# edwindn/rl-agent-for-qubit-array-tuning

Measured on NVIDIA B200. Metric: ground_state_pixels_per_s, higher is better.
Workload: dtype f64

## Files before the change

rl-agent-for-qubit-array-tuning_b200/csrc/qd_api.cu:

```cuda
#include <cuda_runtime.h>
#include <stdarg.h>
#include <stdio.h>
#include <string.h>

#include <new>
#include <stdlib.h>

#include <algorithm>
#include <chrono>
#include <vector>

#include "qd_kernels.cuh"
#include "qd_tunnel.cuh"
#include "qd_tunnel_noda.cuh"
#include "qd_tunnel_enum.cuh"
#include "qd_normalise.cuh"

static_assert(sizeof(qd_scan) == 480, "qd_scan must be 480 bytes (multiple of 16 for the TMA bulk copy)");
static_assert(sizeof(qd_scan) % 16 == 0, "qd_scan size");

struct qd_ctx {
  int device = 0;
  int sm_count = 0;
  char err[512] = {0};
// ... 181 lines not shown
int validate_launch(qd_ctx* ctx, int n_type, unsigned flags, const void* n_out) {
  if (!ctx) return fail(nullptr, QD_ERR_INVALID, "ctx is NULL");
  if (!ctx->have_models) return fail(ctx, QD_ERR_STATE, "qd_set_models has not been called");
  if (n_type < QD_N_NONE || n_type > QD_N_F64) return fail(ctx, QD_ERR_INVALID, "bad n_type %d", n_type);
  if (n_type != QD_N_NONE && !n_out) return fail(ctx, QD_ERR_INVALID, "n_out is NULL but n_type != QD_N_NONE");
  if ((flags & QD_FLAG_THERMAL) && n_type == QD_N_U8)
    return fail(ctx, QD_ERR_INVALID, "QD_FLAG_THERMAL yields non-integer occupations: use QD_N_F32/F64 or QD_N_NONE");
  if ((flags & QD_FLAG_LATCH) && (flags & QD_FLAG_LATCH_EXACT) &&
      ((flags & QD_FLAG_THERMAL) || ctx->L.algorithm == QD_ALG_TUNNEL))
    return fail(ctx, QD_ERR_UNSUPPORTED,
                "QD_FLAG_LATCH_EXACT: exact-compare latching of non-integer occupations (thermal / tunnel path) is not supported");
  if (ctx->L.algorithm == QD_ALG_TUNNEL && n_type == QD_N_U8)
    return fail(ctx, QD_ERR_INVALID, "the tunnel path yields non-integer occupations <n>: use QD_N_F32/F64 or QD_N_NONE");
  return QD_OK;
}

struct KernelConfig { int device; const void* fn; size_t smem; };
KernelConfig g_kernel_config[512];
int g_n_kernel_config = 0;

int configure_kernel(qd_ctx* ctx, const void* fn, size_t smem) {
  int at = -1;
  for (int i = 0; i < g_n_kernel_config; ++i)
    if (g_kernel_config[i].fn == fn && g_kernel_config[i].device == ctx->device) { at = i; break; }
  if (at >= 0 && g_kernel_config[at].smem >= smem) return QD_OK;
  const size_t want = std::max<size_t>(smem, 48 * 1024);
  QD_CUDA(ctx, cudaFuncSetAttribute(fn, cudaFuncAttributeMaxDynamicSharedMemorySize, (int)want));
  if (at < 0) QD_CUDA(ctx, cudaFuncSetAttribute(fn, cudaFuncAttributePreferredSharedMemoryCarveout, 100));
  if (at < 0 && g_n_kernel_config < 512) at = g_n_kernel_config++;
  if (at >= 0) g_kernel_config[at] = KernelConfig{ctx->device, fn, want};
  return QD_OK;
}

int order_after_last_launch(qd_ctx* ctx, cudaStream_t stream) {
  if (ctx->have_last && ctx->last_stream != stream) QD_CUDA(ctx, cudaStreamWaitEvent(stream, ctx->last_launch, 0));
  return QD_OK;
}
int mark_launch(qd_ctx* ctx, cudaStream_t stream) {
  QD_CUDA(ctx, cudaEventRecord(ctx->last_launch, stream));
  ctx->last_stream = stream;
  ctx->have_last = true;
  return QD_OK;
}

int launch(qd_ctx* ctx, int n_scan, const qd_scan* d_scans, int max_ny, const double* d_points, float* d_z, void* d_n,
           int n_type, unsigned flags, cudaStream_t stream, int rows_cap = 0, const qd_scan* h_one = nullptr) {
  {
    const int rc0 = order_after_last_launch(ctx, stream);
    if (rc0) return rc0;
  }
  const bool fast = use_fast_kernel(ctx->L, flags, d_points != nullptr);
  kernel_fn fn = fast ? pick_fast(ctx->L.n_dot) : pick_kernel(ctx->L, flags, d_points != nullptr);
  if (!fn) return fail(ctx, QD_ERR_UNSUPPORTED, "no kernel for n_dot=%d algorithm=%d", ctx->L.n_dot, ctx->L.algorithm);
  qd::KArgs a;
  memset(&a, 0, sizeof(a));
  a.nbar = nullptr;
  if (ctx->L.algorithm == QD_ALG_TUNNEL) {
    const int N = ctx->L.n_dot;
    kernel_fn gs = pick_tunnel_gs(N);
    if (!gs) return fail(ctx, QD_ERR_UNSUPPORTED, "tunnel path needs 2..8 dots, got %d", N);
    int rc = grow(ctx, &ctx->d_nbar, &ctx->nbar_cap, (size_t)ctx->up_pixels * N * sizeof(double));
    if (rc) return rc;
    qd::KArgs g;
    memset(&g, 0, sizeof(g));
    g.L = ctx->L; g.records = ctx->d_records; g.scans = d_scans; g.points = d_points; g.z_out = nullptr;
    g.n_out = nullptr; g.nbar = ctx->d_nbar; g.n_scan = n_scan; g.n_type = QD_N_NONE; g.flags = flags;
    g.status = ctx->d_status;
    g.topt = 7;
    if (const char* e = getenv("QDSIM_TUNNEL_OPT")) g.topt = atoi(e) & 7;
    const long long max_pix = ctx->up_max_pix;
    const char* mono_e = getenv("QDSIM_TUNNEL_MONO");
    const bool mono = mono_e && mono_e[0] == '1';
    if (mono) {
      g.slot_bytes = qd::qd_tunnel_slot_bytes(ctx->L);
      const long long want_items = (long long)ctx->sm_count * 12 * 4;
      long long ppi = ((long long)n_scan * max_pix) / want_items;
      if (ppi < 1) ppi = 1;
      if (ppi > 64) ppi = 64;
      g.rows_per_item = (int)ppi;
      g.items_per_scan = (int)((max_pix + ppi - 1) / ppi);
      const long long items = (long long)n_scan * g.items_per_scan;
      const int gw = (items < (long long)ctx->sm_count * 4) ? 1 : 4;
      long long ggrid = (items + gw - 1) / gw;
      if (ggrid > 0x7fffffffLL) ggrid = 0x7fffffffLL;
      const size_t gsmem = (size_t)g.slot_bytes * gw;
      rc = configure_kernel(ctx, (const void*)gs, gsmem);
      if (rc) return rc;
      gs<<<(unsigned)ggrid, gw * 32, gsmem, stream>>>(g);
      QD_CUDA(ctx, cudaGetLastError());
      ctx->launches += 1;
    } else {
      kernel_fn kr = pick_tunnel_relax(N), ks = pick_tunnel_select(N), ke = pick_tunnel_eigen(N);
      long long chunk_pix = 8LL << 20;
      if (const char* e = getenv("QDSIM_TUNNEL_CHUNK_PIX")) chunk_pix = atoll(e) > 0 ? atoll(e) : chunk_pix;
      long long spc = chunk_pix / max_pix;
      if (spc < 1) spc = 1;
      if (spc > n_scan) spc = n_scan;
      rc = grow(ctx, &ctx->d_tfloor, &ctx->tfloor_cap, (size_t)spc * max_pix * 8);
      if (rc) return rc;
      rc = grow(ctx, &ctx->d_tkeys, &ctx->tkeys_cap, (size_t)spc * max_pix * 256);
      if (rc) return rc;
      rc = grow(ctx, &ctx->d_tpot, &ctx->tpot_cap, (size_t)spc * max_pix * 128);
      if (rc) return rc;
      g.tfloor = ctx->d_tfloor;
      g.tpot = ctx->d_tpot;
      g.tkeys = ctx->d_tkeys;
// ... 800 lines not shown
```

rl-agent-for-qubit-array-tuning_b200/csrc/qd_kernels.cuh:

```cuda
#pragma once
#include <math.h>

#include "qd_device.cuh"
#include "qd_layout.h"

namespace qd {

struct KArgs {
  qd_layout L;
  const double* __restrict__ records;
  const qd_scan* __restrict__ scans;
  const double* __restrict__ points;
  float* __restrict__ z_out;
  void* __restrict__ n_out;
  double* __restrict__ nbar;
  unsigned* status;
  unsigned char* tfloor;
  unsigned long long* tkeys;
  double* tpot;
  long long tstride;
  int topt;
  int fixup;
  int mark_ppi;
  float e2_kappa, e2_qsafe, e2_tol;
// ... 17 lines not shown
  int b = L.rec_doubles * 8 + (int)sizeof(qd_scan) + QD_DER_DOUBLES * 8 + 16;
  if (L.algorithm == QD_ALG_DEFAULT || L.algorithm == QD_ALG_THRESHOLDED) b += QD_PC_DOUBLES * 8;
  if (L.algorithm == QD_ALG_BRUTE_FORCE) b += QD_BF_DOUBLES * 8;
  return (b + 127) & ~127;
}

#ifndef QD_MIN_BLOCKS
#define QD_MIN_BLOCKS 3
#endif
#ifndef QD_CTA_WARPS
#define QD_CTA_WARPS 4
#endif
constexpr int QD_PC_WAYS = 8;

template <int N>
__device__ __forceinline__ void matvec_smem(const double* __restrict__ M, const double (&x)[N], double (&y)[N]) {
  if constexpr (N % 2 == 0) {
#pragma unroll
    for (int i = 0; i < N; ++i) {
      double s0 = 0.0, s1 = 0.0;
#pragma unroll
      for (int j = 0; j < N; j += 2) {
        const double2 m = *reinterpret_cast<const double2*>(M + i * N + j);
        s0 = fma(m.x, x[j], s0);
        s1 = fma(m.y, x[j + 1], s1);
      }
      y[i] = s0 + s1;
    }
  } else {
#pragma unroll
    for (int i = 0; i < N; ++i) {
      double s0 = 0.0;
#pragma unroll
      for (int j = 0; j < N; ++j) s0 = fma(M[i * N + j], x[j], s0);
      y[i] = s0;
    }
  }
}
struct ProjCache {
  double* aff;
  const double* gsrc;
  double* lin_s;
  uint32_t* keys;
  uint32_t* meta;
  double* mats;
  double* aug;
  int mat_stride;
};

template <int N>
__device__ __noinline__ int proj_cache_build(const ProjCache& pc, const double* __restrict__ cdd, unsigned S, int lane) {
  constexpr int W = 2 * N;
  double* A = pc.aug;
  for (int e = lane; e < N * W; e += 32) {
    const int r = e / W, c = e - r * W;
    double v;
    if (c < N) v = (((S >> r) & 1u) && ((S >> c) & 1u)) ? cdd[r * N + c] : (r == c ? 1.0 : 0.0);
    else v = (r == c - N) ? 1.0 : 0.0;
    A[e] = v;
  }
  __syncwarp();
  for (int k = 0; k < N; ++k) {
    if (!((S >> k) & 1u)) continue;
    const double inv = 1.0 / A[k * W + k];
    double rowk[(N * W + 31) / 32], fr[(N * W + 31) / 32];
#pragma unroll
    for (int t = 0; t < (N * W + 31) / 32; ++t) {
      const int e = lane + 32 * t;
      if (e < N * W) {
        const int r = e / W, c = e - r * W;
        rowk[t] = A[k * W + c] * inv;
        fr[t] = A[r * W + k];
      }
    }
    __syncwarp();
#pragma unroll
    for (int t = 0; t < (N * W + 31) / 32; ++t) {
      const int e = lane + 32 * t;
      if (e < N * W) {
        const int r = e / W;
        A[e] = (r == k) ? rowk[t] : A[e] - fr[t] * rowk[t];
      }
    }
    __syncwarp();
  }
  const int slot = (int)pc.meta[1];
  double* P = pc.mats + slot * pc.mat_stride;
  for (int e = lane; e < N * N; e += 32) {
    const int i = e / N, j = e - i * N;
    double v = (i == j) ? 1.0 : 0.0;
    if ((S >> j) & 1u) {
      for (int q = 0; q < N; ++q)
        if ((S >> q) & 1u) v -= cdd[i * N + q] * A[q * W + N + j];
    }
    if ((S >> i) & 1u) v = 0.0;
    P[e] = v;
  }
  __syncwarp();
  if (pc.gsrc != nullptr && lane < 24) {
    const int t = lane >> 3, i = lane & 7;
    double acc = 0.0;
    if (i < N) {
      const double* src = pc.gsrc + 8 * t;
      for (int j = 0; j < N; ++j) acc = fma(P[i * N + j], src[j], acc);
    }
    pc.aff[slot * 24 + lane] = acc;
// ... 466 lines not shown
};
__device__ __forceinline__ ItemWindow item_window(const KArgs& a, int part, int nx, int ny) {
  const int cparts = a.col_parts > 1 ? a.col_parts : 1;
  const int rpart = part / cparts, cpart = part - rpart * cparts;
  ItemWindow w;
  w.row0 = rpart * a.rows_per_item;
  w.row1 = min(ny, w.row0 + a.rows_per_item);
  const int n_chunk_x = (nx + 31) >> 5;
  w.cx0 = ((n_chunk_x * cpart) / cparts) << 5;
  w.cx1 = min(nx, ((n_chunk_x * (cpart + 1)) / cparts) << 5);
  w.empty = w.row0 >= ny || w.cx0 >= w.cx1;
  return w;
}

template <int N>
__device__ __forceinline__ void item_affine_forms(const KArgs& a, const double* rec, const qd_scan* sc, double* der, int lane,
                                                  bool check_overflow = true) {
  const qd_layout& L = a.L;
  const int NV = L.n_volt;
  if (lane <= N) {
    const double* arow = (lane < N) ? rec + L.o_a + lane * NV : rec + L.o_sa;
    double s0 = 0.0, sx = 0.0, sy = 0.0;
    for (int k = 0; k < NV; ++k) {
      const double c = arow[k];
      s0 = fma(c, sc->v0[k], s0);
      sx = fma(c, sc->dx[k], sx);
      sy = fma(c, sc->dy[k], sy);
    }
    if (lane < N) {
      der[lane] = s0; der[8 + lane] = sx; der[16 + lane] = sy;
      const double gmax = s0 + fmax(sx * (double)(sc->nx - 1), 0.0) + fmax(sy * (double)(sc->ny - 1), 0.0);
      const bool replaced = (a.flags & QD_FLAG_RADIAL) && sc->rad_mode == 2;
      if (check_overflow && !replaced && !(gmax < 252.0) && a.status)
        *reinterpret_cast<volatile unsigned*>(a.status) = QD_STATUS_OCC_OVERFLOW;
    } else { der[24] = s0; der[25] = sx; der[26] = sy; }
  }
}

struct PixelDraws {
  float z_white, z_rad, u_latch, u_tele;
};
__device__ __forceinline__ PixelDraws pixel_draws(bool need_rng, uint64_t seed, long long pix) {
  PixelDraws d = {0.f, 0.f, 0.f, 0.f};
  if (need_rng) {
    const Philox4 w = philox4x32_10(seed, (uint64_t)pix, 0u);
    box_muller(w.w0, w.w1, d.z_white, d.z_rad);
    d.u_latch = u24(w.w2);
    d.u_tele = u24(w.w3);
  }
  return d;
}

template <typename TakeHeld>
__device__ __forceinline__ void latch_chunk(uint64_t& key, uint64_t& held_key, unsigned todo, float u_latch, const double* rec,
                                            const qd_layout& L, int lane, TakeHeld&& take_held) {
  while (true) {
    const unsigned diff = __ballot_sync(0xffffffffu, key != held_key) & todo;
    if (!diff) break;
    const int i = __ffs(diff) - 1;
    const uint64_t ck = shfl_u64(key, i);
    const uint64_t x = ck ^ held_key;
    const uint64_t nz = (((x & 0x7f7f7f7f7f7f7f7fULL) + 0x7f7f7f7f7f7f7f7fULL) | x) & 0x8080808080808080ULL;
    const int ndiff = __popcll(nz);
    double p_acc = 2.0;
    if (ndiff == 1) {
      p_acc = rec[L.o_pleads + ((__ffsll((long long)nz) - 1) >> 3)];
    } else if (ndiff == 2) {
      const int d0 = (__ffsll((long long)nz) - 1) >> 3;
      const int d1 = (63 - __clzll((long long)nz)) >> 3;
      p_acc = rec[L.o_pinter + d0 * 8 + d1];
    }
    const unsigned from_i = ~((1u << i) - 1u);
    const unsigned same = __ballot_sync(0xffffffffu, key == ck) & todo & from_i;
    const unsigned brk = ~same & from_i & todo;
    const unsigned run = same & ~(brk ? (~0u << (__ffs(brk) - 1)) : 0u);
    const unsigned acc = __ballot_sync(0xffffffffu, (double)u_latch < p_acc) & run;
    const int acl = acc ? __ffs(acc) - 1 : 32;
    const unsigned rejected = run & ((acl >= 32) ? ~0u : ((1u << acl) - 1u));
    if ((rejected >> lane) & 1u) key = held_key;
    take_held(i, rejected, acl);
    if (acl < 32) held_key = ck;
    const int done_to = (acl < 32) ? acl : (31 - __clz(run));
    todo &= ~((2u << done_to) - 1u);
  }
}

__device__ __forceinline__ uint32_t tele_start(bool f_carry, uint64_t seed, int iy, const double* par) {
  if (f_carry) return 0u;
  const Philox4 wr = philox4x32_10(seed, (uint64_t)iy, 1u);
  return ((double)u24(wr.w0) < par[QD_PAR_TELE_STAT]) ? 1u : 0u;
}

__device__ __forceinline__ float sensor_lorentz10(double x0, double xs) {
  float zs = 0.f;
#pragma unroll
  for (int k = -5; k < 5; ++k) {
    const float xk = (float)fma((double)k, xs, x0);
    zs += rcp_approx(fmaf(xk, xk, 1.0f));
  }
  return zs;
}

__device__ __forceinline__ float radial_amp(const qd_scan* sc, double fx, double fy) {
  const float vx = (float)fma(fx, sc->rad_dx, sc->rad_x0);
  const float vy = (float)fma(fy, sc->rad_dy, sc->rad_y0);
  const float dist = sqrtf(fmaf(vx, vx, vy * vy));
  return fminf(fmaxf((float)sc->rad_alpha * (dist - (float)sc->rad_zero_radius), 0.0f), (float)sc->rad_max_amp);
}

template <int N, int ALG, bool THERMAL, bool POINTS>
__global__ void __launch_bounds__(QD_CTA_WARPS * 32, QD_MIN_BLOCKS) qd_scan_kernel(const KArgs a) {
  extern __shared__ __align__(128) unsigned char qd_smem[];
  const int lane = threadIdx.x & 31;
  const int warp = threadIdx.x >> 5;
  const int warps_per_cta = blockDim.x >> 5;
  const qd_layout& L = a.L;
  const int NV = L.n_volt;

  unsigned char* slot = qd_smem + (size_t)warp * a.slot_bytes;
  double* rec = reinterpret_cast<double*>(slot);
  qd_scan* sc = reinterpret_cast<qd_scan*>(slot + (size_t)L.rec_doubles * 8);
  double* der = reinterpret_cast<double*>(slot + (size_t)L.rec_doubles * 8 + sizeof(qd_scan));
  uint64_t* bar = reinterpret_cast<uint64_t*>(der + QD_DER_DOUBLES);
// ... 118 lines not shown
        if (!replace) {
          if constexpr (!POINTS) {
            const double fx = (double)ixc, fy = (double)iy;
#pragma unroll
            for (int j = 0; j < N; ++j) g[j] = fma(fy, d_gy[j], fma(fx, d_gx[j], d_g0[j]));
            us = fma(fy, d_us[2], fma(fx, d_us[1], d_us[0]));
          } else {
            const double* __restrict__ v = a.points + (size_t)pix * NV;
#pragma unroll
            for (int j = 0; j < N; ++j) g[j] = 0.0;
            us = 0.0;
            for (int k = 0; k < NV; ++k) {
              const double vk = v[k];
#pragma unroll
              for (int j = 0; j < N; ++j) g[j] = fma(rec[L.o_a + j * NV + k], vk, g[j]);
              us = fma(rec[L.o_sa + k], vk, us);
            }
            if constexpr (ALG != QD_ALG_BRUTE_FORCE) {
              bool big = false;
#pragma unroll
              for (int j = 0; j < N; ++j) big |= !(g[j] < 252.0);
              if (big && a.status) *reinterpret_cast<volatile unsigned*>(a.status) = QD_STATUS_OCC_OVERFLOW;
            }
          }

          if constexpr (ALG == QD_ALG_TUNNEL) {
            const double* __restrict__ src = a.nbar + (size_t)(pix0 + pix) * N;
#pragma unroll
            for (int j = 0; j < N; ++j) nd[j] = src[j];
          } else if constexpr (ALG == QD_ALG_BRUTE_FORCE) {
            double gp[N];
            if constexpr (!POINTS) {
              const double fx = (double)ixc, fy = (double)iy;
#pragma unroll
              for (int l = 0; l < N; ++l) { const int j = bf_pm[l]; gp[l] = fma(fy, d_gy[j], fma(fx, d_gx[j], d_g0[j])); }
            } else {
#pragma unroll
              for (int l = 0; l < N; ++l) gp[l] = g[l];
            }
            ground_state_brute<N, THERMAL>(gp, rec, L, bf_ud, bf_pm, kT, nd);
          }
          else ground_state_box<N, THERMAL, !POINTS>(g, rec, L, pc, lane, L.algorithm == QD_ALG_THRESHOLDED, kT, (double)ixc, (double)iy, nd);

          if (latch_on) {
            const bool integral = ALG != QD_ALG_TUNNEL && kT <= 0.0;
            uint64_t key = pack_key<N>(nd, integral);
            const uint64_t key_free = key;
            unsigned todo = vmask;
            if (!have_held) {
              held_key = shfl_u64(key, 0);
              todo &= ~1u;
              have_held = true;
            }
            latch_chunk(key, held_key, todo, rnd.u_latch, rec, L, lane, [&](int i, unsigned rejected, int) {
              if (rejected && !integral) {
                const int src = (i > 0) ? i - 1 : 0;
#pragma unroll
                for (int j = 0; j < N; ++j) {
                  const double prev = shfl_f64(nd[j], src);
                  const double held = (i > 0) ? prev : d_carry[j];
                  if ((rejected >> lane) & 1u) nd[j] = held;
                }
              }
            });
            if (integral) {
              if (key != key_free) {
#pragma unroll
                for (int j = 0; j < N; ++j) nd[j] = (double)(int)((unsigned)(key >> (8 * j)) & 0xffu);
              }
            } else {
              const int last = 31 - __clz(vmask);
              if (lane == last) {
#pragma unroll
                for (int j = 0; j < N; ++j) d_carry[j] = nd[j];
              }
              __syncwarp();
            }
          }

          double noise_in = 0.0, noise_out = 0.0;
          if (f_noise) {
            const double wn = par[QD_PAR_WHITE] * (double)rnd.z_white;
            if (f_white_out) noise_out = wn; else noise_in = wn;
            const double tamp = par[QD_PAR_TELE_AMP];
            if (tamp != 0.0) {
              if (!tele_init) {
                tele_state = tele_start(f_carry, seed, iy, par);
                tele_init = true;
              }
              const uint32_t flip0 = ((double)rnd.u_tele < par[QD_PAR_P01]) ? 1u : 0u;
              const uint32_t flip1 = ((double)rnd.u_tele < par[QD_PAR_P10]) ? 1u : 0u;
              uint32_t fn = valid ? ((0u ^ flip0) | ((1u ^ flip1) << 1)) : 2u;
#pragma unroll
              for (int d = 1; d < 32; d <<= 1) {
                const uint32_t other = __shfl_up_sync(0xffffffffu, fn, d);
                if (lane >= d) fn = compose2(fn, other);
              }
              const uint32_t st = (fn >> tele_state) & 1u;
              tele_state = __shfl_sync(0xffffffffu, st, 31);
              noise_in += tamp * (double)st;
            }
          }
          if (f_pink && par[QD_PAR_PINK] != 0.0) {
            if (!pink_init) {
              const Philox4 ws = philox4x32_10(seed, (uint64_t)iy, 3u);
              float s0, s1, s2, s3;
              box_muller(ws.w0, ws.w1, s0, s1);
// ... 55 lines not shown
            }
            z = zs + noise_out;
          } else {
            z = (double)sensor_lorentz10(x0, xs) + noise_out;
          }
          if (f_radial && sc->rad_mode == 1) z = fma((double)rnd.z_rad, (double)radial_amp(sc, (double)ixc, (double)iy), z);
          zf = (float)z;
        } else {
          zf = rnd.z_rad;
#pragma unroll
          for (int j = 0; j < N; ++j) nd[j] = 0.0;
        }

        if (valid) {
          const long long o = pix0 + (long long)iy * nx + ix;
          if (a.z_out) a.z_out[o] = zf;
          if (a.n_type == QD_N_U8) {
            unsigned char* p = reinterpret_cast<unsigned char*>(a.n_out) + o * N;
            if constexpr (N == 8) {
              uint64_t k = 0;
#pragma unroll
              for (int j = 0; j < N; ++j) k |= (uint64_t)(unsigned char)min(255, (int)nd[j]) << (8 * j);
              *reinterpret_cast<uint64_t*>(p) = k;
            } else if constexpr (N == 4) {
              uint32_t k = 0;
#pragma unroll
              for (int j = 0; j < N; ++j) k |= (uint32_t)(unsigned char)min(255, (int)nd[j]) << (8 * j);
              *reinterpret_cast<uint32_t*>(p) = k;
            } else if constexpr (N == 2) {
              const uint16_t k = (uint16_t)((unsigned char)min(255, (int)nd[0]) | ((unsigned char)min(255, (int)nd[1]) << 8));
              *reinterpret_cast<uint16_t*>(p) = k;
            } else {
#pragma unroll
              for (int j = 0; j < N; ++j) p[j] = (unsigned char)min(255, (int)nd[j]);
            }
          } else if (a.n_type == QD_N_F32) {
            float* p = reinterpret_cast<float*>(a.n_out) + o * N;
#pragma unroll
            for (int j = 0; j < N; ++j) p[j] = (float)nd[j];
          } else if (a.n_type == QD_N_F64) {
            double* p = reinterpret_cast<double*>(a.n_out) + o * N;
#pragma unroll
            for (int j = 0; j < N; ++j) p[j] = nd[j];
          }
        }
      }
    }
    __syncwarp();
  }
}


#ifndef QD_FAST_MIN_BLOCKS
#define QD_FAST_MIN_BLOCKS 4
#endif
constexpr int QD_FAST_DER = 32;
constexpr int QD_FAST_PC = 64 + 8 * 16 + 8 + 8 * 32 + QD_PC_WAYS * 24;

__host__ __device__ inline int qd_fast_slot_bytes(const qd_layout& L) {
  const int b = L.rec_doubles * 8 + (int)sizeof(qd_scan) + (QD_FAST_DER + 32 + QD_FAST_PC) * 8 + 16;
  return (b + 127) & ~127;
}

template <int N>
__global__ void __launch_bounds__(QD_CTA_WARPS * 32, QD_FAST_MIN_BLOCKS) qd_scan_fast_kernel(const KArgs a) {
  extern __shared__ __align__(128) unsigned char qd_smem[];
  const int lane = threadIdx.x & 31;
  const int warp = threadIdx.x >> 5;
  const int warps_per_cta = blockDim.x >> 5;
  const qd_layout& L = a.L;

  unsigned char* slot = qd_smem + (size_t)warp * a.slot_bytes;
  double* rec = reinterpret_cast<double*>(slot);
  qd_scan* sc = reinterpret_cast<qd_scan*>(slot + (size_t)L.rec_doubles * 8);
  double* der = reinterpret_cast<double*>(slot + (size_t)L.rec_doubles * 8 + sizeof(qd_scan));
  double* d_g0 = der;
  double* d_gx = der + 8;
  double* d_gy = der + 16;
  double* d_us = der + 24;
  double* d_sg = der + 27;
  double* swt = der + QD_FAST_DER;
  ProjCache pc;
  pc.mats = swt + 32;
  pc.aug = pc.mats + 64;
  pc.keys = reinterpret_cast<uint32_t*>(pc.aug + 8 * 16);
  pc.meta = pc.keys + QD_PC_WAYS;
  pc.lin_s = pc.aug + 8 * 16 + 8;
  pc.aff = pc.lin_s + 8 * 32;
  pc.gsrc = der;
  pc.mat_stride = 0;
  uint64_t* bar = reinterpret_cast<uint64_t*>(pc.aff + QD_PC_WAYS * 24);

  if (lane == 0) mbar_init(bar, 1);
  __syncwarp();
  uint32_t phase = 0;

  const bool f_latch = a.flags & QD_FLAG_LATCH;
  const bool f_noise = a.flags & QD_FLAG_NOISE;
  const bool f_radial = a.flags & QD_FLAG_RADIAL;
  const bool f_carry = a.flags & QD_FLAG_CARRY_ROWS;
  const bool f_white_out = a.flags & QD_FLAG_WHITE_ON_OUTPUT;
  const bool thresholded = L.algorithm == QD_ALG_THRESHOLDED;
  const uint32_t rec_bytes = (uint32_t)L.rec_doubles * 8u;
  const double* __restrict__ cinv = rec + L.o_cinv;
  const double* __restrict__ Q = rec + L.o_q;
  const double* __restrict__ spos = rec + L.o_spos;
  const double* __restrict__ sneg = rec + L.o_sneg;
  const double* __restrict__ sw = rec + L.o_sw;
  const double* par = rec + L.o_par;

  const long long total_items = (long long)a.n_scan * a.items_per_scan;
  for (long long item = (long long)blockIdx.x * warps_per_cta + warp; item < total_items;
       item += (long long)gridDim.x * warps_per_cta) {
    const int scan_id = (int)(item / a.items_per_scan);
    const int part = (int)(item - (long long)scan_id * a.items_per_scan);
    const qd_scan* gscan = a.scans + scan_id;

    stage_item(a, gscan, rec_bytes, rec, sc, bar, phase, lane, a.use_one);
    if (lane == 0) { pc.meta[0] = 0u; pc.meta[1] = 0u; }

    const int nx = sc->nx, ny = sc->ny;
    const ItemWindow w = item_window(a, part, nx, ny);
    if (w.empty) { __syncwarp(); continue; }
    const int row0 = w.row0, row1 = w.row1, cx0 = w.cx0, cx1 = w.cx1;

    item_affine_forms<N>(a, rec, sc, der, lane);
    {
      double t = 0.0;
      const int h = lane & 15;
#pragma unroll
      for (int q = 0; q < 4; ++q) {
        const int p = (lane < 16) ? q : q + 4;
        if (p < N && ((h >> q) & 1)) t += sw[N - 1 - p];
      }
      swt[lane] = t;
    }
    __syncwarp();
    if (lane < 3) {
      double t = 0.0;
      for (int j = 0; j < N; ++j) t = fma(sw[j], der[8 * lane + j], t);
      d_sg[lane] = t;
    }
    __syncwarp();

    const bool latch_on = f_latch && par[QD_PAR_LATCH] != 0.0;
    const bool replace = f_radial && sc->rad_mode == 2;
    const uint64_t seed = sc->seed;
    const long long pix0 = sc->pix_offset;
    const double inv_gamma = 1.0 / sc->peak_width;
    const double css = rec[L.o_css];
    const bool need_rng = f_noise || latch_on || (f_radial && sc->rad_mode != 0);

    uint64_t held_key = 0;
    double held_sn = 0.0;
    bool have_held = false;
    uint32_t tele_state = 0;
    bool tele_init = false;

    for (int iy = row0; iy < row1; ++iy) {
      if (!f_carry) { have_held = false; tele_init = false; }
      for (int c0 = cx0; c0 < cx1; c0 += 32) {
        const int ix = c0 + lane;
        const bool valid = ix < nx;
        const int ixc = valid ? ix : nx - 1;
        const long long pix = (long long)iy * nx + ixc;
        const unsigned vmask = __ballot_sync(0xffffffffu, valid);
        const double fx = (double)ixc, fy = (double)iy;
        const PixelDraws rnd = pixel_draws(need_rng, seed, pix);

        uint64_t key = 0;
        float zf;
        if (!replace) {
          double sn;
          {
            double g[N], nc[N];
            int sgn = 0;
#pragma unroll
            for (int j = 0; j < N; ++j) {
              g[j] = fma(fy, d_gy[j], fma(fx, d_gx[j], d_g0[j]));
              nc[j] = g[j];
              sgn |= __double2hiint(g[j]);
            }
            if (__any_sync(0xffffffffu, sgn < 0)) relax_lcp<N, true>(g, rec + L.o_cdd, pc, lane, fx, fy, nc);
            double r[N], lin[N];
            unsigned fixmask = 0, fixval = 0;
            uint32_t klo = 0, khi = 0;
            sn = 0.0;
#pragma unroll
            for (int j = 0; j < N; ++j) {
              const double fj = floor(nc[j]);
              r[j] = fj - g[j];
              sn = fma(sw[j], fj, sn);
              const uint32_t fi = (uint32_t)__double2int_rz(fj) & 0xffu;
              if (j < 4) klo |= fi << (8 * j); else khi |= fi << (8 * (j - 4));
              if (thresholded) {
                const double frac = nc[j] - fj;
                if (!(fabs(frac - 0.5) < 0.5 * par[QD_PAR_THRESHOLD])) {
                  fixmask |= 1u << (N - 1 - j);
                  if (floor(nc[j] + 0.5) - fj == 1.0) fixval |= 1u << (N - 1 - j);
                }
              }
            }
            key = ((uint64_t)khi << 32) | klo;
            matvec_smem<N>(cinv, r, lin);
            double* __restrict__ ls = pc.lin_s + lane;
            unsigned zmask = 0, omask = 0;
#pragma unroll
            for (int j = 0; j < N; ++j) {
              const unsigned bit = 1u << (N - 1 - j);
              const double l2 = lin[j] + lin[j];
              ls[(N - 1 - j) * 32] = l2;
              const double aj = l2 + cinv[j * N + j];
              zmask |= (aj + sneg[j] > 1e-9) ? bit : 0u;
              omask |= (aj + spos[j] < -1e-9) ? bit : 0u;
            }
            const unsigned add = (zmask | omask) & ~fixmask;
            fixval |= omask & add;
            fixmask |= add;
            const unsigned freeb = ~fixmask & ((1u << N) - 1u);
            const int kfree = __popc(freeb);
            const int kmax = __reduce_max_sync(0xffffffffu, kfree);
            unsigned idx = fixval;
            double Lsum = 0.0;
#pragma unroll
            for (int p = 0; p < N; ++p)
              if ((fixval >> p) & 1u) Lsum += ls[p * 32];
            double best = Lsum + Q[idx];
            unsigned bidx = idx;
            if (kmax > 0) {
              unsigned pos = 0;
              {
                int nfree = 0;
#pragma unroll
                for (int p = 0; p < N; ++p)
                  if ((freeb >> p) & 1u) { pos |= (unsigned)p << (4 * nfree); ++nfree; }
              }
              const unsigned steps = 1u << kmax, mine = 1u << kfree;
#pragma unroll 1
              for (unsigned c = 1; c < steps; ++c) {
                if (c < mine) {
                  const unsigned p = (pos >> (4 * (__ffs(c) - 1))) & 15u;
                  idx ^= 1u << p;
                  const double lp = ls[p * 32];
                  Lsum += ((idx >> p) & 1u) ? lp : -lp;
                  const double e = Lsum + Q[idx];
                  if (e < best || (e == best && idx < bidx)) { best = e; bidx = idx; }
                }
              }
            }
            key += ((((uint64_t)(bidx << (8 - N))) * 0x8040201008040201ULL) & 0x8080808080808080ULL) >> 7;
            sn += swt[bidx & 15u] + swt[16 + (bidx >> 4)];
          }

          if (latch_on) {
            unsigned todo = vmask;
            if (!have_held) {
              held_key = shfl_u64(key, 0);
              held_sn = shfl_f64(sn, 0);
              todo &= ~1u;
              have_held = true;
            }
            latch_chunk(key, held_key, todo, rnd.u_latch, rec, L, lane, [&](int, unsigned rejected, int acl) {
              if ((rejected >> lane) & 1u) sn = held_sn;
              if (acl < 32) held_sn = shfl_f64(sn, acl);
            });
          }

          double noise_in = 0.0, noise_out = 0.0;
          if (f_noise) {
            const double wn = par[QD_PAR_WHITE] * (double)rnd.z_white;
            if (f_white_out) noise_out = wn; else noise_in = wn;
            const double tamp = par[QD_PAR_TELE_AMP];
            if (tamp != 0.0) {
              if (!tele_init) {
                tele_state = tele_start(f_carry, seed, iy, par);
                tele_init = true;
              }
              const unsigned f0 = __ballot_sync(0xffffffffu, valid && (double)rnd.u_tele < par[QD_PAR_P01]);
              const unsigned f1 = __ballot_sync(0xffffffffu, valid && (double)rnd.u_tele < par[QD_PAR_P10]);
              unsigned st_mask = 0u, rem = 0xffffffffu, cur = tele_state;
              while (true) {
                const unsigned m = (cur ? f1 : f0) & rem;
                if (!m) { if (cur) st_mask |= rem; break; }
                const int t = __ffs(m) - 1;
                if (cur) st_mask |= rem & ((1u << t) - 1u);
                cur ^= 1u;
                if (cur) st_mask |= 1u << t;
                rem &= ~((2u << t) - 1u);
                if (!rem) break;
              }
              tele_state = cur;
              noise_in += tamp * (double)((st_mask >> lane) & 1u);
            }
          }

          const double us = fma(fy, d_us[2], fma(fx, d_us[1], d_us[0]));
          const double sg = fma(fy, d_sg[2], fma(fx, d_sg[1], d_sg[0]));
          const double base = 2.0 * (sn - sg);
          const double t = (rint(us) + noise_in) - us;
          const double xs = 2.0 * css * inv_gamma;
          const double x0 = fma(css, fma(2.0, t, 1.0), base) * inv_gamma;
          double z = (double)sensor_lorentz10(x0, xs) + noise_out;
          if (f_radial && sc->rad_mode == 1) z = fma((double)rnd.z_rad, (double)radial_amp(sc, fx, fy), z);
          zf = (float)z;
        } else {
          zf = rnd.z_rad;
        }

        if (valid) {
          const long long o = pix0 + (long long)iy * nx + ix;
          if (a.z_out) a.z_out[o] = zf;
          if (a.n_type == QD_N_U8) {
            unsigned char* p = reinterpret_cast<unsigned char*>(a.n_out) + o * N;
            if constexpr (N == 8) *reinterpret_cast<uint64_t*>(p) = key;
            else if constexpr (N == 4) *reinterpret_cast<uint32_t*>(p) = (uint32_t)key;
            else if constexpr (N == 2) *reinterpret_cast<uint16_t*>(p) = (uint16_t)key;
            else {
#pragma unroll
              for (int j = 0; j < N; ++j) p[j] = (unsigned char)(key >> (8 * j));
            }
          } else if (a.n_type == QD_N_F32) {
            float* p = reinterpret_cast<float*>(a.n_out) + o * N;
#pragma unroll
            for (int j = 0; j < N; ++j) p[j] = (float)(unsigned)((key >> (8 * j)) & 0xffu);
          } else if (a.n_type == QD_N_F64) {
            double* p = reinterpret_cast<double*>(a.n_out) + o * N;
#pragma unroll
            for (int j = 0; j < N; ++j) p[j] = (double)(unsigned)((key >> (8 * j)) & 0xffu);
          }
        }
      }
    }
    __syncwarp();
  }
}

__global__ void qd_build_q_kernel(qd_layout L, double* __restrict__ records, int n_env) {
  const int n = L.n_dot;
  const int per = 1 << n;
  const long long total = (long long)n_env * per;
  for (long long t = (long long)blockIdx.x * blockDim.x + threadIdx.x; t < total; t += (long long)gridDim.x * blockDim.x) {
    const int env = (int)(t / per);
    const unsigned idx = (unsigned)(t - (long long)env * per);
    double* rec = records + (size_t)env * L.rec_doubles;
    const double* cinv = rec + L.o_cinv;
    double s = 0.0;
    for (int i = 0; i < n; ++i) {
      if (!((idx >> (n - 1 - i)) & 1u)) continue;
      for (int j = 0; j < n; ++j)
        if ((idx >> (n - 1 - j)) & 1u) s += cinv[i * n + j];
    }
    rec[L.o_q + idx] = s;
  }
}

template <typename T>
__global__ void __launch_bounds__(256) qd_fma_peak_kernel(T* out, int iters, T a, T b) {
  T x0 = (T)threadIdx.x, x1 = x0 + 1, x2 = x0 + 2, x3 = x0 + 3, x4 = x0 + 4, x5 = x0 + 5, x6 = x0 + 6, x7 = x0 + 7;
  for (int i = 0; i < iters; ++i) {
#pragma unroll
    for (int u = 0; u < 8; ++u) {
      x0 = x0 * a + b; x1 = x1 * a + b; x2 = x2 * a + b; x3 = x3 * a + b;
      x4 = x4 * a + b; x5 = x5 * a + b; x6 = x6 * a + b; x7 = x7 * a + b;
// ... 7 lines not shown
```

rl-agent-for-qubit-array-tuning_b200/csrc/qd_layout.h:

```cpp
#pragma once
#include <stdint.h>

#include "../../include/qdsim.h"

enum {
  QD_PAR_KT = 0,
  QD_PAR_THRESHOLD = 1,
  QD_PAR_WHITE = 2,
  QD_PAR_P01 = 3,
  QD_PAR_P10 = 4,
  QD_PAR_TELE_AMP = 5,
  QD_PAR_TELE_STAT = 6,
  QD_PAR_LATCH = 7,
  QD_PAR_MAXC = 8,
  QD_PAR_TC_BASE = 9,
  QD_PAR_VC_ALPHA = 10,
  QD_PAR_VC_BETA = 11,
  QD_PAR_PINK = 12,
  QD_PAR_VC_KIND = 13,
  QD_PAR_VC_VCHAR = 14,
  QD_PAR_COUNT = 16
};

struct qd_layout {
  int32_t n_dot, n_volt, n_gate, algorithm;
  int32_t num_states, chunk;
  int32_t o_cinv;
  int32_t o_cdd;
  int32_t o_a;
  int32_t o_sw;
  int32_t o_css;
  int32_t o_sa;
  int32_t o_par;
  int32_t o_alpha;
  int32_t o_pleads;
  int32_t o_pinter;
  int32_t o_spos;
  int32_t o_sneg;
  int32_t o_q;
  int32_t o_cbg;
  int32_t gs_doubles;
  int32_t pad0, pad1;
  int32_t rec_doubles;
};

static inline qd_layout qd_make_layout(int n_dot, int n_volt, int n_gate, int algorithm, int num_states, int chunk) {
  qd_layout L;
  L.n_dot = n_dot; L.n_volt = n_volt; L.n_gate = n_gate; L.algorithm = algorithm;
  L.num_states = num_states; L.chunk = chunk;
  int o = 0;
  L.o_cinv = o;   o += n_dot * n_dot;
  if (algorithm == QD_ALG_TUNNEL) {
    L.o_a = o;      o += n_dot * n_volt;
    L.o_par = o;    o += QD_PAR_COUNT;
    L.o_alpha = o;  o += 8;
    L.o_cbg = o;    o += (n_volt - n_gate) * n_gate;
    o = (o + 1) & ~1;
    L.gs_doubles = o;
    L.o_cdd = o;    o += n_dot * n_dot;
    L.o_sw = o;     o += n_dot;
    L.o_css = o;    o += 1;
    L.o_sa = o;     o += n_volt;
    L.o_pleads = o; o += 8;
    L.o_pinter = o; o += 64;
    L.o_spos = o;   o += 8;
    L.o_sneg = o;   o += 8;
    o = (o + 1) & ~1;
    L.o_q = o;
  } else {
    L.o_cdd = o;    o += n_dot * n_dot;
    L.o_a = o;      o += n_dot * n_volt;
    L.o_sw = o;     o += n_dot;
    L.o_css = o;    o += 1;
    L.o_sa = o;     o += n_volt;
    L.o_par = o;    o += QD_PAR_COUNT;
    L.o_alpha = o;  o += 8;
    L.o_pleads = o; o += 8;
    L.o_pinter = o; o += 64;
    L.o_spos = o;   o += 8;
    L.o_sneg = o;   o += 8;
    o = (o + 1) & ~1;
    L.o_q = o;
    if (algorithm == QD_ALG_DEFAULT || algorithm == QD_ALG_THRESHOLDED) o += (1 << n_dot);
    L.o_cbg = o;
    L.gs_doubles = 0;
  }
  L.pad0 = L.pad1 = 0;
  L.rec_doubles = (o + 1) & ~1;
  return L;
}
```

Before: 15.57 billion.

## Use compile-time record offsets and compact shared-memory slot in fast kernel

Reorders the non-tunnel record layout so the hot fields sit at fixed, n_dot-dependent offsets, which lets the fast kernel index them as compile-time constants and adds a host check that rejects mismatched layouts. The per-warp shared slot is repacked with P/aug overlaid on lin_s to shrink it, and min blocks per SM rises from 4 to 5. The per-pixel cinv*(floor - g) product is split into cinv*floor minus a precomputed affine term (d_hg), using double2 loads, and RNG draws and scan scalars are moved later to lower register pressure. The risks are register spills at the higher occupancy target and slight rounding differences from the reassociated arithmetic.

```diff
diff --git a/rl-agent-for-qubit-array-tuning_b200/csrc/qd_api.cu b/rl-agent-for-qubit-array-tuning_b200/csrc/qd_api.cu
--- a/rl-agent-for-qubit-array-tuning_b200/csrc/qd_api.cu
+++ b/rl-agent-for-qubit-array-tuning_b200/csrc/qd_api.cu
@@ -257,6 +257,8 @@
   const bool fast = use_fast_kernel(ctx->L, flags, d_points != nullptr);
   kernel_fn fn = fast ? pick_fast(ctx->L.n_dot) : pick_kernel(ctx->L, flags, d_points != nullptr);
   if (!fn) return fail(ctx, QD_ERR_UNSUPPORTED, "no kernel for n_dot=%d algorithm=%d", ctx->L.n_dot, ctx->L.algorithm);
+  if (fast && !qd::qd_fast_layout_ok(ctx->L))
+    return fail(ctx, QD_ERR_STATE, "record layout does not match qd_scan_fast_kernel's fixed offsets (n_dot=%d)", ctx->L.n_dot);
   qd::KArgs a;
   memset(&a, 0, sizeof(a));
   a.nbar = nullptr;
diff --git a/rl-agent-for-qubit-array-tuning_b200/csrc/qd_kernels.cuh b/rl-agent-for-qubit-array-tuning_b200/csrc/qd_kernels.cuh
--- a/rl-agent-for-qubit-array-tuning_b200/csrc/qd_kernels.cuh
+++ b/rl-agent-for-qubit-array-tuning_b200/csrc/qd_kernels.cuh
@@ -93,6 +93,7 @@
 __device__ __noinline__ int proj_cache_build(const ProjCache& pc, const double* __restrict__ cdd, unsigned S, int lane) {
   constexpr int W = 2 * N;
   double* A = pc.aug;
+  __syncwarp();
   for (int e = lane; e < N * W; e += 32) {
     const int r = e / W, c = e - r * W;
     double v;
@@ -665,8 +666,8 @@
 }
 
 template <typename TakeHeld>
-__device__ __forceinline__ void latch_chunk(uint64_t& key, uint64_t& held_key, unsigned todo, float u_latch, const double* rec,
-                                            const qd_layout& L, int lane, TakeHeld&& take_held) {
+__device__ __forceinline__ void latch_chunk(uint64_t& key, uint64_t& held_key, unsigned todo, float u_latch,
+                                            const double* p_leads, const double* p_inter, int lane, TakeHeld&& take_held) {
   while (true) {
     const unsigned diff = __ballot_sync(0xffffffffu, key != held_key) & todo;
     if (!diff) break;
@@ -677,11 +678,11 @@
     const int ndiff = __popcll(nz);
     double p_acc = 2.0;
     if (ndiff == 1) {
-      p_acc = rec[L.o_pleads + ((__ffsll((long long)nz) - 1) >> 3)];
+      p_acc = p_leads[(__ffsll((long long)nz) - 1) >> 3];
     } else if (ndiff == 2) {
       const int d0 = (__ffsll((long long)nz) - 1) >> 3;
       const int d1 = (63 - __clzll((long long)nz)) >> 3;
-      p_acc = rec[L.o_pinter + d0 * 8 + d1];
+      p_acc = p_inter[d0 * 8 + d1];
     }
     const unsigned from_i = ~((1u << i) - 1u);
     const unsigned same = __ballot_sync(0xffffffffu, key == ck) & todo & from_i;
@@ -906,7 +907,8 @@
               todo &= ~1u;
               have_held = true;
             }
-            latch_chunk(key, held_key, todo, rnd.u_latch, rec, L, lane, [&](int i, unsigned rejected, int) {
+            latch_chunk(key, held_key, todo, rnd.u_latch, rec + L.o_pleads, rec + L.o_pinter, lane,
+                        [&](int i, unsigned rejected, int) {
               if (rejected && !integral) {
                 const int src = (i > 0) ? i - 1 : 0;
 #pragma unroll
@@ -1068,14 +1070,29 @@
 
 
 #ifndef QD_FAST_MIN_BLOCKS
-#define QD_FAST_MIN_BLOCKS 4
+#define QD_FAST_MIN_BLOCKS 5
 #endif
-constexpr int QD_FAST_DER = 32;
-constexpr int QD_FAST_PC = 64 + 8 * 16 + 8 + 8 * 32 + QD_PC_WAYS * 24;
+constexpr int QD_FAST_O_DER = 0;
+constexpr int QD_FAST_O_HG = 32;
+constexpr int QD_FAST_O_SWT = 56;
+constexpr int QD_FAST_O_KEYS = QD_FAST_O_SWT + 32;
+constexpr int QD_FAST_O_AFF = QD_FAST_O_KEYS + 8;
+constexpr int QD_FAST_O_LIN = QD_FAST_O_AFF + QD_PC_WAYS * 24;
+constexpr int QD_FAST_O_BAR = QD_FAST_O_LIN + 8 * 32;
+constexpr int QD_FAST_O_SCAN = QD_FAST_O_BAR + 2;
+constexpr int QD_FAST_O_REC = QD_FAST_O_SCAN + (int)(sizeof(qd_scan) / 8);
+static_assert(64 + 8 * 16 <= 8 * 32, "P and aug must fit inside lin_s");
+static_assert(sizeof(qd_scan) % 16 == 0 && QD_FAST_O_SCAN % 2 == 0, "TMA destinations must be 16-byte aligned");
 
 __host__ __device__ inline int qd_fast_slot_bytes(const qd_layout& L) {
-  const int b = L.rec_doubles * 8 + (int)sizeof(qd_scan) + (QD_FAST_DER + 32 + QD_FAST_PC) * 8 + 16;
-  return (b + 127) & ~127;
+  return (QD_FAST_O_REC * 8 + L.rec_doubles * 8 + 127) & ~127;
+}
+
+inline bool qd_fast_layout_ok(const qd_layout& L) {
+  const qd_hot_layout H = qd_make_hot_layout(L.n_dot, true);
+  return L.algorithm != QD_ALG_TUNNEL && L.o_cinv == H.cinv && L.o_spos == H.spos && L.o_sneg == H.sneg &&
+         L.o_sw == H.sw && L.o_css == H.css && L.o_par == H.par && L.o_pleads == H.pleads && L.o_pinter == H.pinter &&
+         L.o_q == H.q && L.rec_doubles >= H.end;
 }
 
 template <int N>
@@ -1085,27 +1102,29 @@
   const int warp = threadIdx.x >> 5;
   const int warps_per_cta = blockDim.x >> 5;
   const qd_layout& L = a.L;
-
-  unsigned char* slot = qd_smem + (size_t)warp * a.slot_bytes;
-  double* rec = reinterpret_cast<double*>(slot);
-  qd_scan* sc = reinterpret_cast<qd_scan*>(slot + (size_t)L.rec_doubles * 8);
-  double* der = reinterpret_cast<double*>(slot + (size_t)L.rec_doubles * 8 + sizeof(qd_scan));
-  double* d_g0 = der;
-  double* d_gx = der + 8;
-  double* d_gy = der + 16;
-  double* d_us = der + 24;
+  constexpr qd_hot_layout H = qd_make_hot_layout(N, true);
+
+  double* base = reinterpret_cast<double*>(qd_smem + (size_t)warp * a.slot_bytes);
+  double* rec = base + QD_FAST_O_REC;
+  qd_scan* sc = reinterpret_cast<qd_scan*>(base + QD_FAST_O_SCAN);
+  double* der = base + QD_FAST_O_DER;
+  const double* d_g0 = der;
+  const double* d_gx = der + 8;
+  const double* d_gy = der + 16;
+  const double* d_us = der + 24;
   double* d_sg = der + 27;
-  double* swt = der + QD_FAST_DER;
+  double* d_hg = base + QD_FAST_O_HG;
+  double* swt = base + QD_FAST_O_SWT;
   ProjCache pc;
-  pc.mats = swt + 32;
-  pc.aug = pc.mats + 64;
-  pc.keys = reinterpret_cast<uint32_t*>(pc.aug + 8 * 16);
+  pc.keys = reinterpret_cast<uint32_t*>(base + QD_FAST_O_KEYS);
   pc.meta = pc.keys + QD_PC_WAYS;
-  pc.lin_s = pc.aug + 8 * 16 + 8;
-  pc.aff = pc.lin_s + 8 * 32;
+  pc.aff = base + QD_FAST_O_AFF;
+  pc.lin_s = base + QD_FAST_O_LIN;
+  pc.mats = pc.lin_s;
+  pc.aug = pc.lin_s + 64;
   pc.gsrc = der;
   pc.mat_stride = 0;
-  uint64_t* bar = reinterpret_cast<uint64_t*>(pc.aff + QD_PC_WAYS * 24);
+  uint64_t* bar = reinterpret_cast<uint64_t*>(base + QD_FAST_O_BAR);
 
   if (lane == 0) mbar_init(bar, 1);
   __syncwarp();
@@ -1118,12 +1137,12 @@
   const bool f_white_out = a.flags & QD_FLAG_WHITE_ON_OUTPUT;
   const bool thresholded = L.algorithm == QD_ALG_THRESHOLDED;
   const uint32_t rec_bytes = (uint32_t)L.rec_doubles * 8u;
-  const double* __restrict__ cinv = rec + L.o_cinv;
-  const double* __restrict__ Q = rec + L.o_q;
-  const double* __restrict__ spos = rec + L.o_spos;
-  const double* __restrict__ sneg = rec + L.o_sneg;
-  const double* __restrict__ sw = rec + L.o_sw;
-  const double* par = rec + L.o_par;
+  const double* cinv = rec + H.cinv;
+  const double* Q = rec + H.q;
+  const double* spos = rec + H.spos;
+  const double* sneg = rec + H.sneg;
+  const double* sw = rec + H.sw;
+  const double* par = rec + H.par;
 
   const long long total_items = (long long)a.n_scan * a.items_per_scan;
   for (long long item = (long long)blockIdx.x * warps_per_cta + warp; item < total_items;
@@ -1157,14 +1176,18 @@
       for (int j = 0; j < N; ++j) t = fma(sw[j], der[8 * lane + j], t);
       d_sg[lane] = t;
     }
+    if (lane < 24 && (lane & 7) < N) {
+      const int t = lane >> 3, i = lane & 7;
+      double acc = 0.0;
+      for (int k = 0; k < N; ++k) acc = fma(cinv[i * N + k], der[8 * t + k], acc);
+      d_hg[lane] = acc;
+    }
     __syncwarp();
 
     const bool latch_on = f_latch && par[QD_PAR_LATCH] != 0.0;
     const bool replace = f_radial && sc->rad_mode == 2;
-    const uint64_t seed = sc->seed;
-    const long long pix0 = sc->pix_offset;
-    const double inv_gamma = 1.0 / sc->peak_width;
-    const double css = rec[L.o_css];
+    if (lane == 0) der[30] = 1.0 / sc->peak_width;
+    __syncwarp();
     const bool need_rng = f_noise || latch_on || (f_radial && sc->rad_mode != 0);
 
     uint64_t held_key = 0;
@@ -1182,7 +1205,6 @@
         const long long pix = (long long)iy * nx + ixc;
         const unsigned vmask = __ballot_sync(0xffffffffu, valid);
         const double fx = (double)ixc, fy = (double)iy;
-        const PixelDraws rnd = pixel_draws(need_rng, seed, pix);
 
         uint64_t key = 0;
         float zf;
@@ -1198,14 +1220,14 @@
               sgn |= __double2hiint(g[j]);
             }
             if (__any_sync(0xffffffffu, sgn < 0)) relax_lcp<N, true>(g, rec + L.o_cdd, pc, lane, fx, fy, nc);
-            double r[N], lin[N];
+            double f[N];
             unsigned fixmask = 0, fixval = 0;
             uint32_t klo = 0, khi = 0;
             sn = 0.0;
 #pragma unroll
             for (int j = 0; j < N; ++j) {
               const double fj = floor(nc[j]);
-              r[j] = fj - g[j];
+              f[j] = fj;
               sn = fma(sw[j], fj, sn);
               const uint32_t fi = (uint32_t)__double2int_rz(fj) & 0xffu;
               if (j < 4) klo |= fi << (8 * j); else khi |= fi << (8 * (j - 4));
@@ -1218,13 +1240,28 @@
               }
             }
             key = ((uint64_t)khi << 32) | klo;
-            matvec_smem<N>(cinv, r, lin);
             double* __restrict__ ls = pc.lin_s + lane;
             unsigned zmask = 0, omask = 0;
 #pragma unroll
             for (int j = 0; j < N; ++j) {
               const unsigned bit = 1u << (N - 1 - j);
-              const double l2 = lin[j] + lin[j];
+              double cf;
+              if constexpr (N % 2 == 0) {
+                double s0 = 0.0, s1 = 0.0;
+#pragma unroll
+                for (int k = 0; k < N; k += 2) {
+                  const double2 m = *reinterpret_cast<const double2*>(cinv + j * N + k);
+                  s0 = fma(m.x, f[k], s0);
+                  s1 = fma(m.y, f[k + 1], s1);
+                }
+                cf = s0 + s1;
+              } else {
+                cf = 0.0;
+#pragma unroll
+                for (int k = 0; k < N; ++k) cf = fma(cinv[j * N + k], f[k], cf);
+              }
+              const double hj = cf - fma(fy, d_hg[16 + j], fma(fx, d_hg[8 + j], d_hg[j]));
+              const double l2 = hj + hj;
               ls[(N - 1 - j) * 32] = l2;
               const double aj = l2 + cinv[j * N + j];
               zmask |= (aj + sneg[j] > 1e-9) ? bit : 0u;
@@ -1268,6 +1305,7 @@
             sn += swt[bidx & 15u] + swt[16 + (bidx >> 4)];
           }
 
+          const PixelDraws rnd = pixel_draws(need_rng, sc->seed, pix);
           if (latch_on) {
             unsigned todo = vmask;
             if (!have_held) {
@@ -1276,7 +1314,8 @@
               todo &= ~1u;
               have_held = true;
             }
-            latch_chunk(key, held_key, todo, rnd.u_latch, rec, L, lane, [&](int, unsigned rejected, int acl) {
+            latch_chunk(key, held_key, todo, rnd.u_latch, rec + H.pleads, rec + H.pinter, lane,
+                        [&](int, unsigned rejected, int acl) {
               if ((rejected >> lane) & 1u) sn = held_sn;
               if (acl < 32) held_sn = shfl_f64(sn, acl);
             });
@@ -1289,7 +1328,7 @@
             const double tamp = par[QD_PAR_TELE_AMP];
             if (tamp != 0.0) {
               if (!tele_init) {
-                tele_state = tele_start(f_carry, seed, iy, par);
+                tele_state = tele_start(f_carry, sc->seed, iy, par);
                 tele_init = true;
               }
               const unsigned f0 = __ballot_sync(0xffffffffu, valid && (double)rnd.u_tele < par[QD_PAR_P01]);
@@ -1314,17 +1353,18 @@
           const double sg = fma(fy, d_sg[2], fma(fx, d_sg[1], d_sg[0]));
           const double base = 2.0 * (sn - sg);
           const double t = (rint(us) + noise_in) - us;
+          const double css = rec[H.css], inv_gamma = der[30];
           const double xs = 2.0 * css * inv_gamma;
           const double x0 = fma(css, fma(2.0, t, 1.0), base) * inv_gamma;
           double z = (double)sensor_lorentz10(x0, xs) + noise_out;
           if (f_radial && sc->rad_mode == 1) z = fma((double)rnd.z_rad, (double)radial_amp(sc, fx, fy), z);
           zf = (float)z;
         } else {
-          zf = rnd.z_rad;
+          zf = pixel_draws(need_rng, sc->seed, pix).z_rad;
         }
 
         if (valid) {
-          const long long o = pix0 + (long long)iy * nx + ix;
+          const long long o = sc->pix_offset + (long long)iy * nx + ix;
           if (a.z_out) a.z_out[o] = zf;
           if (a.n_type == QD_N_U8) {
             unsigned char* p = reinterpret_cast<unsigned char*>(a.n_out) + o * N;
diff --git a/rl-agent-for-qubit-array-tuning_b200/csrc/qd_layout.h b/rl-agent-for-qubit-array-tuning_b200/csrc/qd_layout.h
--- a/rl-agent-for-qubit-array-tuning_b200/csrc/qd_layout.h
+++ b/rl-agent-for-qubit-array-tuning_b200/csrc/qd_layout.h
@@ -44,6 +44,33 @@
   int32_t rec_doubles;
 };
 
+#ifdef __CUDACC__
+#define QD_HD __host__ __device__
+#else
+#define QD_HD
+#endif
+
+struct qd_hot_layout {
+  int cinv, spos, sneg, sw, css, par, pleads, pinter, q, end;
+};
+QD_HD constexpr qd_hot_layout qd_make_hot_layout(int n_dot, bool with_q) {
+  qd_hot_layout H{};
+  int o = 0;
+  H.cinv = o;    o += n_dot * n_dot;
+  H.spos = o;    o += 8;
+  H.sneg = o;    o += 8;
+  H.sw = o;      o += n_dot;
+  H.css = o;     o += 1;
+  o = (o + 1) & ~1;
+  H.par = o;     o += QD_PAR_COUNT;
+  H.pleads = o;  o += 8;
+  H.pinter = o;  o += 64;
+  H.q = o;
+  if (with_q) o += 1 << n_dot;
+  H.end = o;
+  return H;
+}
+
 static inline qd_layout qd_make_layout(int n_dot, int n_volt, int n_gate, int algorithm, int num_states, int chunk) {
   qd_layout L;
   L.n_dot = n_dot; L.n_volt = n_volt; L.n_gate = n_gate; L.algorithm = algorithm;
@@ -68,20 +95,20 @@
     o = (o + 1) & ~1;
     L.o_q = o;
   } else {
+    const qd_hot_layout H = qd_make_hot_layout(n_dot, algorithm == QD_ALG_DEFAULT || algorithm == QD_ALG_THRESHOLDED);
+    L.o_spos = H.spos;
+    L.o_sneg = H.sneg;
+    L.o_sw = H.sw;
+    L.o_css = H.css;
+    L.o_par = H.par;
+    L.o_pleads = H.pleads;
+    L.o_pinter = H.pinter;
+    L.o_q = H.q;
+    o = H.end;
+    L.o_alpha = o;  o += 8;
     L.o_cdd = o;    o += n_dot * n_dot;
     L.o_a = o;      o += n_dot * n_volt;
-    L.o_sw = o;     o += n_dot;
-    L.o_css = o;    o += 1;
     L.o_sa = o;     o += n_volt;
-    L.o_par = o;    o += QD_PAR_COUNT;
-    L.o_alpha = o;  o += 8;
-    L.o_pleads = o; o += 8;
-    L.o_pinter = o; o += 64;
-    L.o_spos = o;   o += 8;
-    L.o_sneg = o;   o += 8;
-    o = (o + 1) & ~1;
-    L.o_q = o;
-    if (algorithm == QD_ALG_DEFAULT || algorithm == QD_ALG_THRESHOLDED) o += (1 << n_dot);
     L.o_cbg = o;
     L.gs_doubles = 0;
   }
```

After: 15.02 billion, median of 6. 0.965x the previous value.
